# yml-bit/CTA-GAN

Hardware: AMD Instinct MI355X
Metric: paired 512x512 slices/sec (G+D step); generator rel-L2 vs CPU reference (higher is better)
Workload: dtype bf16; 1 GPU; HdGan stage-2 full G+D train step (G, Reg, STN, D_m, losses, Adam x3), 16 paired 512x512 slices/GPU; per_gpu_batch=16, global_batch=16, size=512, parallelism=single, rccl_ranks=1, dp_backend=none

## Files before the change

cta_gan_amd/csrc/conv_small.hip:

```cpp
#include <stdlib.h>
#include "common.h"
#include "ctg_knobs.h"

struct SmallArgs {
    const float* s0;
    const float* s1;
    const void* w;
    const float* bias;
    void* y;
    float* stats;
    int B, Hi, Wi, Cin, kh, kw, stride, pad, pad_mode;
    int Ho, Wo, Cout, y_ld, act, Kreal, ntiles;
};

#define SMALL_PREF 5

template <typename T, int KPAD, int BN, bool PO = false, bool X3 = false, bool KXW = false>
__global__ __launch_bounds__(256) void conv_small_kernel(const SmallArgs a) {
    static_assert(!KXW || (KPAD == 64 && sizeof(T) == 2), "kx-window layout: 8 kernel rows x 8 columns of bf16");
    static_assert(!PO || sizeof(T) == 4 || X3, "split-pair output: the fp32 or the split-bf16 instantiation");
    static_assert(!X3 || (sizeof(T) == 2 && PO), "split-bf16 MFMA: bf16 tiles, split-pair result");
    constexpr int EPC = VecOf<T>::N;
    constexpr int CPR = KPAD / EPC;
    constexpr int KCH = X3 ? 8 : (CPR < 8 ? CPR : 8);
    constexpr int NSUB = X3 ? KPAD / 32 : CPR / KCH;
    constexpr int CPRW = X3 ? 2 * CPR : CPR;
    constexpr int TM = 4, TN = BN / 16;
    constexpr int PPI = 256 / CPR;
    constexpr int A_BYTES = 256 * KPAD * (int)sizeof(T) * (X3 ? 2 : 1);
    constexpr int ST_BYTES = PO ? 256 * (BN * 4 + 16) : sizeof(T) == 2 ? 256 * (BN * 2 + 16) : 4 * BN * 2 * 4;
    constexpr int A_REGION = A_BYTES > ST_BYTES ? A_BYTES : ST_BYTES;
    typedef T OutT;
    extern __shared__ __attribute__((aligned(16))) char smem[];

    const int tid = threadIdx.x, lane = tid & 63, wave = tid >> 6;
    const int n = blockIdx.y;
    const int tx_n = (a.Wo + 15) >> 4;
    const int PH = 15 * a.stride + a.kh, PW = 15 * a.stride + a.kw;
    const int plane = PH * PW;
    const int patch_elems = a.Cin * plane;

    char* sA = smem;
    char* sW = smem + A_REGION;
    float* patch = reinterpret_cast<float*>(sW + BN * CPRW * 16);

    const int wg = xcd_contiguous(blockIdx.x, gridDim.x);
    const int q = a.ntiles / (int)gridDim.x, rem = a.ntiles % (int)gridDim.x;
    const int t_begin = wg * q + (wg < rem ? wg : rem);
    const int t_end = t_begin + q + (wg < rem ? 1 : 0);
    if (t_begin >= t_end) return;

    {
        const T* W = (const T*)a.w;
        for (int i = tid; i < BN * CPRW; i += 256) {
            const int row = i / CPRW, kc = i - row * CPRW;
            const int sub = kc / KCH, kcl = kc - sub * KCH;
            *reinterpret_cast<u32x4*>(sW + ((sub * BN + row) * KCH + swz<KCH>(row, kcl)) * 16) =
                *reinterpret_cast<const u32x4*>(W + (size_t)row * (CPRW * EPC) + kc * EPC);
        }
    }
    int pe_yx[SMALL_PREF];
#pragma unroll
    for (int j = 0; j < SMALL_PREF; ++j) {
        const int i = tid + 256 * j;
        const int c = i / plane, r = i - c * plane;
        const int py = r / PW, px = r - py * PW;
        pe_yx[j] = i < patch_elems ? (c << 30) | (py << 15) | px : -1;
    }
    float pre[SMALL_PREF];
    unsigned pre_ok = 0;
    auto fetch_patch = [&](int sp) __attribute__((always_inline)) {
        const int iy0 = (sp / tx_n) * 16 * a.stride - a.pad, ix0 = (sp % tx_n) * 16 * a.stride - a.pad;
#pragma unroll
        for (int j = 0; j < SMALL_PREF; ++j) {
            const int e = pe_yx[j];
            int iy = iy0 + ((e >> 15) & 0x7fff), ix = ix0 + (e & 0x7fff);
            if (a.pad_mode == PAD_REFLECT) { iy = reflect_idx(iy, a.Hi); ix = reflect_idx(ix, a.Wi); }
            const bool ok = e >= 0 && (unsigned)iy < (unsigned)a.Hi && (unsigned)ix < (unsigned)a.Wi;
            const float* src = (ok && ((e >> 30) & 1)) ? a.s1 : a.s0;
            const int off = ok ? iy * a.Wi + ix : 0;
            pre[j] = src[(size_t)n * a.Hi * a.Wi + off];
            pre_ok = ok ? (pre_ok | (1u << j)) : (pre_ok & ~(1u << j));
        }
    };
    const int kc = tid % CPR;
    int koff[EPC];
    unsigned kvalid = 0;
#pragma unroll
    for (int e = 0; e < EPC; ++e) {
        const int k = kc * EPC + e;
        const int kk = a.kh * a.kw;
        const int c = k / kk, r = k - c * kk;
        const int ky = r / a.kw, kx = r - ky * a.kw;
        koff[e] = k < a.Kreal ? (c * PH + ky) * PW + kx : 0;
        kvalid |= (k < a.Kreal ? 1u : 0u) << e;
    }
    const int co_l = (lane >> 4) * 4;
    OutT* __restrict__ Y = (OutT*)a.y;
    const float nslope = a.act == ACT_RELU ? 0.f : a.act == ACT_LRELU ? LRELU_SLOPE : 1.f;
    const bool raw = a.bias == nullptr && a.act == ACT_NONE;

    float bv[TN][4];
#pragma unroll
    for (int nt = 0; nt < TN; ++nt)
#pragma unroll
        for (int r = 0; r < 4; ++r) {
            const int co = nt * 16 + co_l + r;
            bv[nt][r] = (a.bias != nullptr && co < a.Cout) ? a.bias[co] : 0.f;
        }

    auto stash_patch = [&]() __attribute__((always_inline)) {
#pragma unroll
        for (int j = 0; j < SMALL_PREF; ++j)
            if (pe_yx[j] >= 0) patch[tid + 256 * j] = ((pre_ok >> j) & 1u) ? pre[j] : 0.f;
    };
    fetch_patch(t_begin);
    stash_patch();
    for (int sp = t_begin; sp < t_end; ++sp) {
        const int y0 = (sp / tx_n) * 16, x0 = (sp % tx_n) * 16;
        lds_barrier();
        if (sp + 1 < t_end) fetch_patch(sp + 1);
        if constexpr (KXW) {
            const int ky = tid & 7, grp = tid >> 3;
            const int r = grp >> 1, xh = (grp & 1) * 8;
            const bool row_ok = ky < a.kh;
            const float* prow = patch + (r + ky) * PW + xh;
            float win[16];
#pragma unroll
            for (int j = 0; j < 15; ++j) win[j] = (row_ok && j < a.kw + 7) ? prow[j] : 0.f;
            win[15] = 0.f;
            const int sub = X3 ? ky >> 2 : 0, kcl = X3 ? ky & 3 : ky;
#pragma unroll
            for (int pp = 0; pp < 8; ++pp) {
                const int p = r * 16 + xh + pp;
                float v[8];
#pragma unroll
                for (int e = 0; e < 8; ++e) v[e] = e < a.kw ? win[pp + e] : 0.f;
                if constexpr (X3) {
                    bf16x8 hi, lo;
#pragma unroll
                    for (int e = 0; e < 8; ++e) {
                        hi[e] = (bf16_t)v[e];
                        lo[e] = (bf16_t)(v[e] - (float)hi[e]);
                    }
                    *reinterpret_cast<bf16x8*>(sA + ((sub * 256 + p) * KCH + swz<KCH>(p, kcl)) * 16) = hi;
                    *reinterpret_cast<bf16x8*>(sA + ((sub * 256 + p) * KCH + swz<KCH>(p, kcl + 4)) * 16) = lo;
                } else {
                    bf16x8 o;
#pragma unroll
                    for (int e = 0; e < 8; ++e) o[e] = (bf16_t)v[e];
                    *reinterpret_cast<bf16x8*>(sA + ((sub * 256 + p) * KCH + swz<KCH>(p, kcl)) * 16) = o;
                }
            }
        } else {
            const int sub = X3 ? kc / 4 : kc / KCH, kcl = X3 ? kc & 3 : kc - sub * KCH;
#pragma unroll 2
            for (int it = 0; it < CPR; ++it) {
                const int p = tid / CPR + it * PPI;
                const int base = ((p >> 4) * a.stride) * PW + (p & 15) * a.stride;
                Chunk<T> o;
#pragma unroll
                for (int e = 0; e < EPC; ++e) {
                    const float v = patch[base + koff[e]];
                    o.v[e] = ((kvalid >> e) & 1u) ? v : 0.f;
                }
                if constexpr (X3) {
                    bf16x8 hi, lo;
#pragma unroll
                    for (int e = 0; e < 8; ++e) {
                        hi[e] = (bf16_t)o.v[e];
                        lo[e] = (bf16_t)(o.v[e] - (float)hi[e]);
                    }
                    *reinterpret_cast<bf16x8*>(sA + ((sub * 256 + p) * KCH + swz<KCH>(p, kcl)) * 16) = hi;
                    *reinterpret_cast<bf16x8*>(sA + ((sub * 256 + p) * KCH + swz<KCH>(p, kcl + 4)) * 16) = lo;
                } else {
                    o.store(reinterpret_cast<T*>(sA + ((sub * 256 + p) * KCH + swz<KCH>(p, kcl)) * 16));
                }
            }
        }
        lds_barrier();

        f32x4 acc[TM][TN];
#pragma unroll
        for (int i = 0; i < TM; ++i)
#pragma unroll
            for (int j = 0; j < TN; ++j) acc[i][j] = f32x4{0.f, 0.f, 0.f, 0.f};
#pragma unroll
        for (int sub = 0; sub < NSUB; ++sub) {
            if constexpr (X3) {
                const int c4 = lane >> 4;
                u32x4 fa[TM], fb[TN], fl[TN];
#pragma unroll
                for (int mt = 0; mt < TM; ++mt) {
                    const int row = (wave * TM + mt) * 16 + (lane & 15);
                    fa[mt] = *reinterpret_cast<const u32x4*>(sA + ((sub * 256 + row) * KCH + swz<KCH>(row, c4)) * 16);
                }
#pragma unroll
                for (int nt = 0; nt < TN; ++nt) {
                    const int row = nt * 16 + (lane & 15);
                    fb[nt] = *reinterpret_cast<const u32x4*>(sW + ((sub * BN + row) * KCH + swz<KCH>(row, c4)) * 16);
                    fl[nt] = *reinterpret_cast<const u32x4*>(sW + ((sub * BN + row) * KCH + swz<KCH>(row, c4 + 4)) * 16);
                }
#pragma unroll
                for (int mt = 0; mt < TM; ++mt)
#pragma unroll
                    for (int nt = 0; nt < TN; ++nt) {
                        acc[mt][nt] = __builtin_amdgcn_mfma_f32_16x16x32_bf16(
                            __builtin_bit_cast(bf16x8, fb[nt]), __builtin_bit_cast(bf16x8, fa[mt]), acc[mt][nt], 0, 0, 0);
                        acc[mt][nt] = __builtin_amdgcn_mfma_f32_16x16x32_bf16(
                            __builtin_bit_cast(bf16x8, fl[nt]), __builtin_bit_cast(bf16x8, fa[mt]), acc[mt][nt], 0, 0, 0);
                    }
#pragma unroll
                for (int mt = 0; mt < TM; ++mt) {
                    const int row = (wave * TM + mt) * 16 + (lane & 15);
                    fa[mt] = *reinterpret_cast<const u32x4*>(sA + ((sub * 256 + row) * KCH + swz<KCH>(row, c4 + 4)) * 16);
                }
#pragma unroll
                for (int mt = 0; mt < TM; ++mt)
#pragma unroll
                    for (int nt = 0; nt < TN; ++nt)
                        acc[mt][nt] = __builtin_amdgcn_mfma_f32_16x16x32_bf16(
                            __builtin_bit_cast(bf16x8, fb[nt]), __builtin_bit_cast(bf16x8, fa[mt]), acc[mt][nt], 0, 0, 0);
            } else
#pragma unroll
            for (int ks = 0; ks < KCH / 4; ++ks) {
                const int c4 = ks * 4 + (lane >> 4);
                u32x4 fa[TM], fb[TN];
#pragma unroll
                for (int mt = 0; mt < TM; ++mt) {
                    const int row = (wave * TM + mt) * 16 + (lane & 15);
                    fa[mt] = *reinterpret_cast<const u32x4*>(sA + ((sub * 256 + row) * KCH + swz<KCH>(row, c4)) * 16);
                }
#pragma unroll
                for (int nt = 0; nt < TN; ++nt) {
                    const int row = nt * 16 + (lane & 15);
                    fb[nt] = *reinterpret_cast<const u32x4*>(sW + ((sub * BN + row) * KCH + swz<KCH>(row, c4)) * 16);
                }
#pragma unroll
                for (int mt = 0; mt < TM; ++mt)
#pragma unroll
                    for (int nt = 0; nt < TN; ++nt) {
                        if constexpr (sizeof(T) == 2) {
                            acc[mt][nt] = __builtin_amdgcn_mfma_f32_16x16x32_bf16(
                                __builtin_bit_cast(bf16x8, fb[nt]), __builtin_bit_cast(bf16x8, fa[mt]), acc[mt][nt], 0, 0, 0);
                        } else {
                            const f32x4 va = __builtin_bit_cast(f32x4, fa[mt]);
                            const f32x4 vb = __builtin_bit_cast(f32x4, fb[nt]);
#pragma unroll
                            for (int qq = 0; qq < 4; ++qq)
                                acc[mt][nt] = __builtin_amdgcn_mfma_f32_16x16x4f32(vb[qq], va[qq], acc[mt][nt], 0, 0, 0);
                        }
                    }
            }
        }
        if (sp + 1 < t_end) stash_patch();
        lds_barrier();

        if (a.stats != nullptr) {
            float* red = reinterpret_cast<float*>(smem);
#pragma unroll
            for (int nt = 0; nt < TN; ++nt) {
                float s1[4] = {0.f, 0.f, 0.f, 0.f}, s2[4] = {0.f, 0.f, 0.f, 0.f};
#pragma unroll
                for (int mt = 0; mt < TM; ++mt) {
                    const bool valid = (y0 + wave * TM + mt < a.Ho) && (x0 + (lane & 15) < a.Wo);
#pragma unroll
                    for (int r = 0; r < 4; ++r) {
                        const float v = valid ? acc[mt][nt][r] : 0.f;
                        s1[r] += v;
                        s2[r] += v * v;
                    }
                }
#pragma unroll
                for (int r = 0; r < 4; ++r) {
                    s1[r] = row16_sum_to_lane15(s1[r]);
                    s2[r] = row16_sum_to_lane15(s2[r]);
                    if ((lane & 15) == 15) {
                        const int cl = nt * 16 + co_l + r;
                        red[(wave * BN + cl) * 2] = s1[r];
                        red[(wave * BN + cl) * 2 + 1] = s2[r];
                    }
                }
            }
            lds_barrier();
            if (tid < BN && tid < a.Cout) {
                float t1 = 0.f, t2 = 0.f;
#pragma unroll
                for (int w = 0; w < 4; ++w) { t1 += red[(w * BN + tid) * 2]; t2 += red[(w * BN + tid) * 2 + 1]; }
                float* dst = a.stats + (((size_t)n * a.ntiles + sp) * a.Cout + tid) * 2;
                dst[0] = t1;
                dst[1] = t2;
            }
            lds_barrier();
        }
        if constexpr (sizeof(OutT) == 2 && !PO) {
            constexpr int RS = BN * 2 + 16;
            char* st = smem;
#pragma unroll
            for (int nt = 0; nt < TN; ++nt) {
                const int co = nt * 16 + co_l;
#pragma unroll
                for (int mt = 0; mt < TM; ++mt) {
                    const int prow = (wave * TM + mt) * 16 + (lane & 15);
                    bf16x4 o;
                    if (raw) {
#pragma unroll
                        for (int r = 0; r < 4; ++r) o[r] = (bf16_t)acc[mt][nt][r];
                    } else {
#pragma unroll
                        for (int r = 0; r < 4; ++r) {
                            const float v = acc[mt][nt][r] + bv[nt][r];
                            o[r] = (bf16_t)(v > 0.f ? v : v * nslope);
                        }
                    }
                    *reinterpret_cast<bf16x4*>(st + prow * RS + co * 2) = o;
                }
            }
            lds_barrier();
            constexpr int CPO = BN / 8;
#pragma unroll
            for (int it = 0; it < CPO; ++it) {
                const int cidx = tid + 256 * it;
                const int prow = cidx / CPO, ch = (cidx % CPO) * 8;
                const int oy = y0 + (prow >> 4), ox = x0 + (prow & 15);
                if (oy < a.Ho && ox < a.Wo && ch < a.Cout)
                    *reinterpret_cast<u32x4*>(Y + (((size_t)n * a.Ho + oy) * a.Wo + ox) * a.y_ld + ch) =
                        *reinterpret_cast<const u32x4*>(st + prow * RS + ch * 2);
            }
        } else if constexpr (PO) {
            constexpr int RS = BN * 4 + 16;
            char* st = smem;
#pragma unroll
            for (int nt = 0; nt < TN; ++nt) {
                const int co = nt * 16 + co_l;
#pragma unroll
                for (int mt = 0; mt < TM; ++mt) {
                    const int prow = (wave * TM + mt) * 16 + (lane & 15);
                    f32x4 o;
                    if (raw) {
                        o = acc[mt][nt];
                    } else {
#pragma unroll
                        for (int r = 0; r < 4; ++r) {
                            const float v = acc[mt][nt][r] + bv[nt][r];
                            o[r] = v > 0.f ? v : v * nslope;
                        }
                    }
                    *reinterpret_cast<f32x4*>(st + prow * RS + co * 4) = o;
                }
            }
            lds_barrier();
            bf16_t* __restrict__ Yp = (bf16_t*)a.y;
            const int y_lo = a.y_ld >> 1;
            constexpr int CPO = BN / 8;
#pragma unroll
            for (int it = 0; it < CPO; ++it) {
                const int cidx = tid + 256 * it;
                const int prow = cidx / CPO, ch = (cidx % CPO) * 8;
                const int oy = y0 + (prow >> 4), ox = x0 + (prow & 15);
                if (oy < a.Ho && ox < a.Wo && ch < a.Cout) {
                    const f32x4 v0 = *reinterpret_cast<const f32x4*>(st + prow * RS + ch * 4);
                    const f32x4 v1 = *reinterpret_cast<const f32x4*>(st + prow * RS + ch * 4 + 16);
                    bf16x8 hi, lo;
#pragma unroll
                    for (int e = 0; e < 4; ++e) {
                        hi[e] = (bf16_t)v0[e];
                        lo[e] = (bf16_t)(v0[e] - (float)hi[e]);
                        hi[4 + e] = (bf16_t)v1[e];
                        lo[4 + e] = (bf16_t)(v1[e] - (float)hi[4 + e]);
                    }
                    bf16_t* yp = Yp + (((size_t)n * a.Ho + oy) * a.Wo + ox) * a.y_ld + ch;
                    *reinterpret_cast<bf16x8*>(yp) = hi;
                    *reinterpret_cast<bf16x8*>(yp + y_lo) = lo;
                }
            }
        } else {
#pragma unroll
            for (int mt = 0; mt < TM; ++mt) {
                const int oy = y0 + wave * TM + mt, ox = x0 + (lane & 15);
                if (oy >= a.Ho || ox >= a.Wo) continue;
                OutT* yp = Y + (((size_t)n * a.Ho + oy) * a.Wo + ox) * a.y_ld;
#pragma unroll
                for (int nt = 0; nt < TN; ++nt) {
                    const int co = nt * 16 + co_l;
                    if (co >= a.Cout) continue;
                    f32x4 v;
#pragma unroll
                    for (int r = 0; r < 4; ++r) {
                        const float t = acc[mt][nt][r] + bv[nt][r];
                        v[r] = t > 0.f ? t : t * nslope;
                    }
                    *reinterpret_cast<f32x4*>(yp + co) = v;
                }
            }
        }
    }
}

template <typename T, int KPAD, int BN, bool PO = false, bool X3 = false, bool KXW = false>
static int launch_small(SmallArgs& a, hipStream_t st, int* tiles_out) {
    const int PH = 15 * a.stride + a.kh, PW = 15 * a.stride + a.kw;
    if (a.Cin * PH * PW > SMALL_PREF * 256 || PH >= 32768 || PW >= 32768) return CTG_EINVAL;
    const int a_bytes = 256 * KPAD * (int)sizeof(T) * (X3 ? 2 : 1);
    const int st_bytes = PO ? 256 * (BN * 4 + 16) : sizeof(T) == 2 ? 256 * (BN * 2 + 16) : 4 * BN * 2 * 4;
    const int smem = (a_bytes > st_bytes ? a_bytes : st_bytes) + BN * KPAD * (int)sizeof(T) * (X3 ? 2 : 1) + (a.Cin * PH * PW + 4) * 4;
    if (smem > 160 * 1024) return CTG_EINVAL;
    static unsigned long long attr_mask = 0;
    if (smem > 64 * 1024) {
        const int rc = ctg_lds_attr_once((const void*)conv_small_kernel<T, KPAD, BN, PO, X3, KXW>, 160 * 1024, &attr_mask);
        if (rc != CTG_OK) return rc;
    }
    const int tiles = ((a.Ho + 15) / 16) * ((a.Wo + 15) / 16);
    a.ntiles = tiles;
    if (tiles_out != nullptr) *tiles_out = tiles;
    const int wg_total = ctg_knobs().small_wgs;
    int gx = (wg_total + a.B - 1) / a.B;
    if (gx > tiles) gx = tiles;
    hipLaunchKernelGGL((conv_small_kernel<T, KPAD, BN, PO, X3, KXW>), dim3(gx, a.B), dim3(256), smem, st, a);
    return ctg_launch_status();
}

extern "C" int ctg_conv_smallcin(int dtype, const float* s0, const float* s1, int Cin, int B, int Hi, int Wi, int kh,
                                 int kw, int stride, int pad, int pad_mode, const void* w, int w_npad, int Kpad, int w_layout,
                                 const float* bias, int act, void* y, int y_ld, int Ho, int Wo, int Cout,
                                 float* stats_part, int* stats_slabs_out, void* stream) {
    CTG_ENTER();
    if (w_layout != 0 && (w_layout != 1 || Cin != 1 || stride != 1 || kh > 8 || kw > 8 || Kpad != 64 || Cout <= 32 ||
                          dtype == DT_F32)) return CTG_EINVAL;
    if (dtype != DT_F32 && dtype != DT_BF16 && dtype != DT_PAIR) return CTG_EINVAL;
    const bool pair = dtype == DT_PAIR;
    if (pair && (Cout % 8 || y_ld % 16 || y_ld < 2 * Cout)) return CTG_EINVAL;
    const int epc = dtype == DT_BF16 ? 8 : 4;
    if (Cin < 1 || Cin > 2 || (Cin == 2 && s1 == nullptr) || s0 == nullptr || w == nullptr || y == nullptr) return CTG_EINVAL;
    if (B < 1 || kh < 1 || kw < 1 || stride < 1 || stride > 2 || pad < 0) return CTG_EINVAL;
    if (act != ACT_NONE && act != ACT_RELU && act != ACT_LRELU) return CTG_EINVAL;
    if ((w_layout == 0 && Cin * kh * kw > Kpad) || (Kpad != 32 && Kpad != 64)) return CTG_EINVAL;
    if (Cout < 1 || Cout > 64 || Cout % epc || y_ld % epc || y_ld < Cout) return CTG_EINVAL;
    if (pad_mode == PAD_REFLECT && (pad >= Hi || pad >= Wi)) return CTG_EINVAL;
    if (Ho != (Hi + 2 * pad - kh) / stride + 1 || Wo != (Wi + 2 * pad - kw) / stride + 1 || Ho < 1 || Wo < 1) return CTG_EINVAL;
    const int bn = Cout > 32 ? 64 : 32;
    if (w_npad < bn) return CTG_EINVAL;
    if (((uintptr_t)w & 15) || ((uintptr_t)y & 15)) return CTG_EINVAL;
    SmallArgs a;
    a.s0 = s0; a.s1 = s1; a.w = w; a.bias = bias; a.y = y; a.stats = stats_part;
    a.B = B; a.Hi = Hi; a.Wi = Wi; a.Cin = Cin; a.kh = kh; a.kw = kw; a.stride = stride; a.pad = pad;
    a.pad_mode = pad_mode; a.Ho = Ho; a.Wo = Wo; a.Cout = Cout; a.y_ld = y_ld; a.act = act; a.Kreal = Cin * kh * kw;
    hipStream_t st = (hipStream_t)stream;
    int tiles = 0, rc;
    if (w_layout == 1) {
        rc = pair ? launch_small<bf16_t, 64, 64, true, true, true>(a, st, &tiles) : launch_small<bf16_t, 64, 64, false, false, true>(a, st, &tiles);
    } else if (dtype == DT_BF16) {
        if (Kpad == 64) rc = bn == 64 ? launch_small<bf16_t, 64, 64>(a, st, &tiles) : launch_small<bf16_t, 64, 32>(a, st, &tiles);
        else rc = bn == 64 ? launch_small<bf16_t, 32, 64>(a, st, &tiles) : launch_small<bf16_t, 32, 32>(a, st, &tiles);
    } else if (pair) {
        if (Kpad == 64) rc = bn == 64 ? launch_small<bf16_t, 64, 64, true, true>(a, st, &tiles) : launch_small<bf16_t, 64, 32, true, true>(a, st, &tiles);
        else rc = bn == 64 ? launch_small<bf16_t, 32, 64, true, true>(a, st, &tiles) : launch_small<bf16_t, 32, 32, true, true>(a, st, &tiles);
    } else {
        if (Kpad == 64) rc = bn == 64 ? launch_small<float, 64, 64>(a, st, &tiles) : launch_small<float, 64, 32>(a, st, &tiles);
        else rc = bn == 64 ? launch_small<float, 32, 64>(a, st, &tiles) : launch_small<float, 32, 32>(a, st, &tiles);
    }
    if (stats_slabs_out != nullptr) *stats_slabs_out = stats_part != nullptr ? tiles : 0;
    return rc;
}
```

cta_gan_amd/csrc/loss_stn.hip:

```cpp
#include "common.h"

static inline int ew_blocks(long items) {
    long b = (items + 255) / 256;
    return (int)(b < 1 ? 1 : (b > 4096 ? 4096 : b));
}

__device__ __forceinline__ void block_partial(float v, float* __restrict__ part) {
    __shared__ float ws[4];
    v = wave_sum(v);
    if ((threadIdx.x & 63) == 0) ws[threadIdx.x >> 6] = v;
    __syncthreads();
    if (threadIdx.x == 0) part[blockIdx.x] = (ws[0] + ws[1]) + (ws[2] + ws[3]);
}

__global__ __launch_bounds__(256) void sum_finalize_kernel(const float* __restrict__ part, int n, float scale,
                                                           float* __restrict__ out, int accumulate) {
    __shared__ double ws[4];
    double s = 0.0;
    for (int i = threadIdx.x; i < n; i += 256) s += (double)part[i];
#pragma unroll
    for (int o = 32; o > 0; o >>= 1) s += __shfl_xor(s, o, 64);
    if ((threadIdx.x & 63) == 0) ws[threadIdx.x >> 6] = s;
    __syncthreads();
    if (threadIdx.x == 0) {
        const float r = (float)(((ws[0] + ws[1]) + (ws[2] + ws[3])) * (double)scale);
        out[0] = accumulate ? out[0] + r : r;
    }
}

struct WarpGeom {
    float iy, ix, my, mx;
};

__device__ __forceinline__ void warp_coord(float g, float f, int size, float& c, float& mult) {
    const float sm1 = (float)(size - 1);
    float loc = g + f;
    loc = 2.f * (loc / sm1 - 0.5f);
    float u = ((loc + 1.f) / 2.f) * sm1;
    float m = sm1 / 2.f;
    if (u <= 0.f) { u = 0.f; m = 0.f; }
    else if (u >= sm1) { u = sm1; m = 0.f; }
    c = u;
    mult = (m * 2.f) / sm1;
}

__global__ void warp_fwd_kernel(const float* __restrict__ src, const float* __restrict__ flow, long fs_n, long fs_c,
                                long fs_y, long fs_x, float* __restrict__ out, int B, int H, int W) {
    const long total = (long)B * H * W;
    for (long i = (long)blockIdx.x * blockDim.x + threadIdx.x; i < total; i += (long)gridDim.x * blockDim.x) {
        const int x = (int)(i % W);
        const int y = (int)((i / W) % H);
        const int n = (int)(i / ((long)W * H));
        const float* fl = flow + n * fs_n + y * fs_y + x * fs_x;
        float iy, ix, my, mx;
        warp_coord((float)y, fl[0], H, iy, my);
        warp_coord((float)x, fl[fs_c], W, ix, mx);
        const float fy = floorf(iy), fx = floorf(ix);
        const int y0 = (int)fy, x0 = (int)fx, y1 = y0 + 1, x1 = x0 + 1;
        const float nw = ((fx + 1.f) - ix) * ((fy + 1.f) - iy), ne = (ix - fx) * ((fy + 1.f) - iy);
        const float sw = ((fx + 1.f) - ix) * (iy - fy), se = (ix - fx) * (iy - fy);
        const float* s = src + (size_t)n * H * W;
        float r = s[(size_t)y0 * W + x0] * nw;
        if (x1 < W) r += s[(size_t)y0 * W + x1] * ne;
        if (y1 < H) r += s[(size_t)y1 * W + x0] * sw;
        if (y1 < H && x1 < W) r += s[(size_t)y1 * W + x1] * se;
        out[i] = r;
    }
}

__global__ void zero_f32_kernel(float* __restrict__ p, long n) {
    for (long i = (long)blockIdx.x * blockDim.x + threadIdx.x; i < n; i += (long)gridDim.x * blockDim.x) p[i] = 0.f;
}

__global__ void warp_bwd_kernel(const float* __restrict__ src, const float* __restrict__ flow, long fs_n, long fs_c,
                                long fs_y, long fs_x, const float* __restrict__ gout, float* __restrict__ dsrc,
                                float* __restrict__ dflow, int B, int H, int W) {
    const long total = (long)B * H * W;
    for (long i = (long)blockIdx.x * blockDim.x + threadIdx.x; i < total; i += (long)gridDim.x * blockDim.x) {
        const int x = (int)(i % W);
        const int y = (int)((i / W) % H);
        const int n = (int)(i / ((long)W * H));
        const long fo = n * fs_n + y * fs_y + x * fs_x;
        float iy, ix, my, mx;
        warp_coord((float)y, flow[fo], H, iy, my);
        warp_coord((float)x, flow[fo + fs_c], W, ix, mx);
        const float fy = floorf(iy), fx = floorf(ix);
        const int y0 = (int)fy, x0 = (int)fx, y1 = y0 + 1, x1 = x0 + 1;
        const float wx1 = ix - fx, wx0 = (fx + 1.f) - ix, wy1 = iy - fy, wy0 = (fy + 1.f) - iy;
        const float g = gout[i];
        const float* s = src + (size_t)n * H * W;
        float* ds = dsrc ? dsrc + (size_t)n * H * W : nullptr;
        const bool bx = x1 < W, by = y1 < H;
        const float vnw = s[(size_t)y0 * W + x0];
        const float vne = bx ? s[(size_t)y0 * W + x1] : 0.f;
        const float vsw = by ? s[(size_t)y1 * W + x0] : 0.f;
        const float vse = (bx && by) ? s[(size_t)y1 * W + x1] : 0.f;
        if (ds) {
            atomicAdd(ds + (size_t)y0 * W + x0, wx0 * wy0 * g);
            if (bx) atomicAdd(ds + (size_t)y0 * W + x1, wx1 * wy0 * g);
            if (by) atomicAdd(ds + (size_t)y1 * W + x0, wx0 * wy1 * g);
            if (bx && by) atomicAdd(ds + (size_t)y1 * W + x1, wx1 * wy1 * g);
        }
        if (dflow) {
            const float gix = (-vnw * wy0 + vne * wy0 - vsw * wy1 + vse * wy1) * g;
            const float giy = (-vnw * wx0 - vne * wx1 + vsw * wx0 + vse * wx1) * g;
            dflow[fo] = my * giy;
            dflow[fo + fs_c] = mx * gix;
        }
    }
}

__global__ void warp_det_prep_kernel(const float* __restrict__ gout, long long* __restrict__ acc, unsigned* __restrict__ maxbits,
                                     long n) {
    unsigned m = 0u;
    for (long i = (long)blockIdx.x * blockDim.x + threadIdx.x; i < n; i += (long)gridDim.x * blockDim.x) {
        acc[i] = 0;
        const unsigned b = __float_as_uint(gout[i]) & 0x7fffffffu;
        m = b > m ? b : m;
    }
#pragma unroll
    for (int o = 32; o > 0; o >>= 1) {
        const unsigned t = (unsigned)__shfl_xor((int)m, o, 64);
        m = t > m ? t : m;
    }
    if ((threadIdx.x & 63) == 0 && m) atomicMax(maxbits, m);
}

__device__ __forceinline__ float det_scale(unsigned maxbits, bool inverse) {
    int e = (int)(maxbits >> 23) - 127;
    e = e < -88 ? -88 : (e > 88 ? 88 : e);
    return __uint_as_float((unsigned)((inverse ? e - 38 : 38 - e) + 127) << 23);
}

__global__ void warp_bwd_det_kernel(const float* __restrict__ flow, long fs_n, long fs_c, long fs_y, long fs_x,
                                    const float* __restrict__ gout, long long* __restrict__ acc,
                                    const unsigned* __restrict__ maxbits, int B, int H, int W) {
    const long total = (long)B * H * W;
    const float sc = det_scale(maxbits[0], false);
    for (long i = (long)blockIdx.x * blockDim.x + threadIdx.x; i < total; i += (long)gridDim.x * blockDim.x) {
        const int x = (int)(i % W);
        const int y = (int)((i / W) % H);
        const int n = (int)(i / ((long)W * H));
        const long fo = n * fs_n + y * fs_y + x * fs_x;
        float iy, ix, my, mx;
        warp_coord((float)y, flow[fo], H, iy, my);
        warp_coord((float)x, flow[fo + fs_c], W, ix, mx);
        const float fy = floorf(iy), fx = floorf(ix);
        const int y0 = (int)fy, x0 = (int)fx, y1 = y0 + 1, x1 = x0 + 1;
        const float wx1 = ix - fx, wx0 = (fx + 1.f) - ix, wy1 = iy - fy, wy0 = (fy + 1.f) - iy;
        const float g = gout[i] * sc;
        unsigned long long* ds = reinterpret_cast<unsigned long long*>(acc + (size_t)n * H * W);
        const bool bx = x1 < W, by = y1 < H;
        atomicAdd(ds + (size_t)y0 * W + x0, (unsigned long long)__float2ll_rn(wx0 * wy0 * g));
        if (bx) atomicAdd(ds + (size_t)y0 * W + x1, (unsigned long long)__float2ll_rn(wx1 * wy0 * g));
        if (by) atomicAdd(ds + (size_t)y1 * W + x0, (unsigned long long)__float2ll_rn(wx0 * wy1 * g));
        if (bx && by) atomicAdd(ds + (size_t)y1 * W + x1, (unsigned long long)__float2ll_rn(wx1 * wy1 * g));
    }
}

__global__ void warp_det_finish_kernel(const long long* __restrict__ acc, const unsigned* __restrict__ maxbits,
                                       float* __restrict__ dsrc, long n) {
    const float inv = det_scale(maxbits[0], true);
    for (long i = (long)blockIdx.x * blockDim.x + threadIdx.x; i < n; i += (long)gridDim.x * blockDim.x)
        dsrc[i] = (float)acc[i] * inv;
}

__global__ void smooth_fwd_kernel(const float* __restrict__ f, long sn, long sc, long sy, long sx, int B, int C,
                                  int H, int W, float inv_nx, float inv_ny, float* __restrict__ part) {
    const long total = (long)B * C * H * W;
    float acc = 0.f;
    for (long i = (long)blockIdx.x * blockDim.x + threadIdx.x; i < total; i += (long)gridDim.x * blockDim.x) {
        const int x = (int)(i % W);
        const int y = (int)((i / W) % H);
        const int c = (int)((i / ((long)W * H)) % C);
        const int n = (int)(i / ((long)W * H * C));
        const float* p = f + n * sn + c * sc + y * sy + x * sx;
        const float v = p[0];
        if (x + 1 < W) { const float d = p[sx] - v; acc += d * d * inv_nx; }
        if (y + 1 < H) { const float d = p[sy] - v; acc += d * d * inv_ny; }
    }
    block_partial(acc, part);
}

__global__ void smooth_bwd_kernel(const float* __restrict__ f, long sn, long sc, long sy, long sx, int B, int C,
                                  int H, int W, float inv_nx, float inv_ny, const float* __restrict__ gscale,
                                  float* __restrict__ df, int accumulate) {
    const long total = (long)B * C * H * W;
    const float g = gscale[0];
    for (long i = (long)blockIdx.x * blockDim.x + threadIdx.x; i < total; i += (long)gridDim.x * blockDim.x) {
        const int x = (int)(i % W);
        const int y = (int)((i / W) % H);
        const int c = (int)((i / ((long)W * H)) % C);
        const int n = (int)(i / ((long)W * H * C));
        const long o = n * sn + c * sc + y * sy + x * sx;
        const float v = f[o];
        float r = 0.f;
        if (x + 1 < W) r -= 2.f * (f[o + sx] - v) * inv_nx;
        if (x > 0) r += 2.f * (v - f[o - sx]) * inv_nx;
        if (y + 1 < H) r -= 2.f * (f[o + sy] - v) * inv_ny;
        if (y > 0) r += 2.f * (v - f[o - sy]) * inv_ny;
        df[o] = accumulate ? df[o] + g * r : g * r;
    }
}

__device__ __forceinline__ float l1_term(float a, float b, const float* mask, long i, float& dsign) {
    if (mask == nullptr) {
        const float d = a - b;
        dsign = d > 0.f ? 1.f : (d < 0.f ? -1.f : 0.f);
        return fabsf(d);
    }
    const float bb = mask[i] < 0.3f ? 0.f : 1.f;
    float bm = b * bb;
    if (bm == 0.f) bm = -1.f;
    const float ab = a * bb;
    const float am = ab == 0.f ? -1.f : ab;
    const float d = am - bm;
    dsign = ab == 0.f ? 0.f : bb * (d > 0.f ? 1.f : (d < 0.f ? -1.f : 0.f));
    return fabsf(d);
}

__global__ void l1_fwd_kernel(const float* __restrict__ a, const float* __restrict__ b,
                              const float* __restrict__ mask, long n, float* __restrict__ part) {
    float acc = 0.f;
    for (long i = (long)blockIdx.x * blockDim.x + threadIdx.x; i < n; i += (long)gridDim.x * blockDim.x) {
        float ds;
        acc += l1_term(a[i], b[i], mask, i, ds);
    }
    block_partial(acc, part);
}

__global__ void l1_bwd_kernel(const float* __restrict__ a, const float* __restrict__ b,
                              const float* __restrict__ mask, long n, const float* __restrict__ gscale, float inv_n,
                              float* __restrict__ da, int accumulate) {
    const float g = gscale[0] * inv_n;
    for (long i = (long)blockIdx.x * blockDim.x + threadIdx.x; i < n; i += (long)gridDim.x * blockDim.x) {
        float ds;
        l1_term(a[i], b[i], mask, i, ds);
        da[i] = accumulate ? da[i] + g * ds : g * ds;
    }
}

__global__ void avgpool_fwd_kernel(const float* __restrict__ x, int HW, float* __restrict__ out) {
    __shared__ float ws[4];
    const int n = blockIdx.x;
    float acc = 0.f;
    for (int i = threadIdx.x; i < HW; i += blockDim.x) acc += x[(size_t)n * HW + i];
    acc = wave_sum(acc);
    if ((threadIdx.x & 63) == 0) ws[threadIdx.x >> 6] = acc;
    __syncthreads();
    if (threadIdx.x == 0) out[n] = ((ws[0] + ws[1]) + (ws[2] + ws[3])) / (float)HW;
}

__global__ void avgpool_bwd_kernel(const float* __restrict__ gout, int HW, float* __restrict__ dx, long total) {
    for (long i = (long)blockIdx.x * blockDim.x + threadIdx.x; i < total; i += (long)gridDim.x * blockDim.x)
        dx[i] = gout[i / HW] / (float)HW;
}

__device__ __forceinline__ double gan_term(double p, double t, int mode) {
    if (mode == 0) return (p - t) * (p - t);
    const double lp = fmax(log(p), -100.0), lq = fmax(log(1.0 - p), -100.0);
    return -(t * lp + (1.0 - t) * lq);
}
__device__ __forceinline__ float gan_term_grad(float p, float t, int mode) {
    if (mode == 0) return 2.f * (p - t);
    return (p - t) / fmaxf(p * (1.f - p), 1e-12f);
}

__global__ __launch_bounds__(256) void lsgan_finalize_kernel(const float* __restrict__ pooled, int B, int nb, float t0,
                                                             float s0, float t1, float s1, int mode,
                                                             float* __restrict__ out) {
    __shared__ double ws[4];
    double s = 0.0;
    for (int b = threadIdx.x; b < B; b += 256)
        s += (double)(b < nb ? s0 : s1) * gan_term((double)pooled[b], (double)(b < nb ? t0 : t1), mode);
#pragma unroll
    for (int o = 32; o > 0; o >>= 1) s += __shfl_xor(s, o, 64);
    if ((threadIdx.x & 63) == 0) ws[threadIdx.x >> 6] = s;
    __syncthreads();
    if (threadIdx.x == 0) out[0] = (float)((ws[0] + ws[1]) + (ws[2] + ws[3]));
}

__global__ void lsgan_bwd_kernel(const float* __restrict__ pooled, int HW, int nb, float t0, float s0, float t1, float s1,
                                 int mode, const float* __restrict__ gscale, float* __restrict__ dx, long total) {
    const float g = gscale[0] / (float)HW;
    for (long i = (long)blockIdx.x * blockDim.x + threadIdx.x; i < total; i += (long)gridDim.x * blockDim.x) {
        const int b = (int)(i / HW);
        dx[i] = g * (b < nb ? s0 : s1) * gan_term_grad(pooled[b], b < nb ? t0 : t1, mode);
    }
}

struct ScalarList { const float* p[8]; int n; };
__global__ void sum_scalars_kernel(const ScalarList L, float* __restrict__ out) {
    float s = 0.f;
    for (int i = 0; i < L.n; ++i) s += L.p[i][0];
    out[0] = s;
}

__global__ void act_bwd_sum_kernel(const float* __restrict__ g, const float* __restrict__ y, int act,
                                   float* __restrict__ out, long n, float* __restrict__ part) {
    float acc = 0.f;
    for (long i = (long)blockIdx.x * blockDim.x + threadIdx.x; i < n; i += (long)gridDim.x * blockDim.x) {
        const float v = g[i] * act_grad_from_out(y[i], act);
        out[i] = v;
        acc += v;
    }
    block_partial(acc, part);
}

template <typename T>
__global__ void weight_pack_kernel(const float* __restrict__ src, long sn, long sk, long stp, int Nreal, int Kreal,
                                   T* __restrict__ dst, int ntaps, int Npad, int Kpad) {
    const long total = (long)ntaps * Npad * Kpad;
    for (long i = (long)blockIdx.x * blockDim.x + threadIdx.x; i < total; i += (long)gridDim.x * blockDim.x) {
        const int k = (int)(i % Kpad);
        const int n = (int)((i / Kpad) % Npad);
        const int t = (int)(i / ((long)Kpad * Npad));
        const float v = (n < Nreal && k < Kreal) ? src[n * sn + k * sk + t * stp] : 0.f;
        st1(dst + i, v);
    }
}

#define PACK_MAX_T 24
struct PackList {
    const float* src[PACK_MAX_T];
    void* dst[PACK_MAX_T];
    long sn[PACK_MAX_T], sk[PACK_MAX_T], stp[PACK_MAX_T];
    int nreal[PACK_MAX_T], kreal[PACK_MAX_T], ntaps[PACK_MAX_T], npad[PACK_MAX_T], kpad[PACK_MAX_T];
    int first[PACK_MAX_T + 1];
    int count;
};
#define PACK_CHUNK 2048

template <typename T>
__global__ __launch_bounds__(256) void weight_pack_multi_kernel(const PackList L) {
    int j = 0;
    while (j + 1 < L.count && (int)blockIdx.x >= L.first[j + 1]) ++j;
    const int Kpad = L.kpad[j], Npad = L.npad[j], Nreal = L.nreal[j], Kreal = L.kreal[j];
    const long sn = L.sn[j], sk = L.sk[j], stp = L.stp[j];
    const float* __restrict__ src = L.src[j];
    T* __restrict__ dst = (T*)L.dst[j];
    const unsigned total = (unsigned)L.ntaps[j] * Npad * Kpad;
    const unsigned base = ((unsigned)blockIdx.x - L.first[j]) * PACK_CHUNK;
#pragma unroll 2
    for (unsigned e = threadIdx.x; e < PACK_CHUNK; e += 256) {
        const unsigned i = base + e;
        if (i >= total) break;
        const unsigned k = i % (unsigned)Kpad, r = i / (unsigned)Kpad;
        const unsigned n = r % (unsigned)Npad, t = r / (unsigned)Npad;
        const float v = ((int)n < Nreal && (int)k < Kreal) ? src[n * sn + k * sk + t * stp] : 0.f;
        st1(dst + i, v);
    }
}

#define ADAM_MAX_T 24
struct AdamList {
    float* p[ADAM_MAX_T];
    const float* g[ADAM_MAX_T];
    float* m[ADAM_MAX_T];
    float* v[ADAM_MAX_T];
    int n[ADAM_MAX_T];
    int count;
};
#define ADAM_CHUNK 4096

__global__ __launch_bounds__(256) void adam_kernel(const AdamList L, float lr, float b1, float b2, float eps,
                                                   float bc1, float bc2_sqrt, const float* __restrict__ dev_bc) {
    if (dev_bc != nullptr) {
        bc1 = dev_bc[1];
        bc2_sqrt = dev_bc[2];
    }
    const int t = blockIdx.y;
    if (t >= L.count) return;
    const int n = L.n[t];
    const int beg = blockIdx.x * ADAM_CHUNK;
    if (beg >= n) return;
    const int end = min(beg + ADAM_CHUNK, n);
    float* __restrict__ p = L.p[t];
    const float* __restrict__ g = L.g[t];
    float* __restrict__ m = L.m[t];
    float* __restrict__ v = L.v[t];
    const float step = lr / bc1;
    for (int i = beg + threadIdx.x; i < end; i += 256) {
        const float gi = g[i];
        float mi = m[i], vi = v[i];
        mi = mi + (gi - mi) * (1.f - b1);
        vi = vi * b2 + (1.f - b2) * gi * gi;
        const float denom = sqrtf(vi) / bc2_sqrt + eps;
        p[i] = p[i] - step * (mi / denom);
        m[i] = mi;
        v[i] = vi;
    }
}

__global__ void adam_tick_kernel(float* __restrict__ state, float b1, float b2) {
    if (threadIdx.x == 0 && blockIdx.x == 0) {
        const double step = (double)state[0] + 1.0;
        state[0] = (float)step;
        state[1] = (float)(1.0 - pow((double)b1, step));
        state[2] = (float)sqrt(1.0 - pow((double)b2, step));
    }
}

extern "C" int ctg_warp_fwd(const float* src, const float* flow, long fs_n, long fs_c, long fs_y, long fs_x,
                            float* out, int B, int H, int W, void* stream) {
    CTG_ENTER();
    if (H < 2 || W < 2) return CTG_EINVAL;
    hipLaunchKernelGGL(warp_fwd_kernel, dim3(ew_blocks((long)B * H * W)), dim3(256), 0, (hipStream_t)stream, src,
                       flow, fs_n, fs_c, fs_y, fs_x, out, B, H, W);
    return ctg_launch_status();
}

extern "C" int ctg_warp_bwd(const float* src, const float* flow, long fs_n, long fs_c, long fs_y, long fs_x,
                            const float* gout, float* dsrc, float* dflow, int B, int H, int W, void* det_ws, void* stream) {
    CTG_ENTER();
    if (H < 2 || W < 2) return CTG_EINVAL;
    hipStream_t st = (hipStream_t)stream;
    if (dsrc && det_ws) {
        if ((uintptr_t)det_ws & 7) return CTG_EINVAL;
        const long n = (long)B * H * W;
        long long* acc = (long long*)det_ws;
        unsigned* maxbits = (unsigned*)(acc + n);
        hipLaunchKernelGGL(zero_f32_kernel, dim3(1), dim3(64), 0, st, (float*)maxbits, 2L);
        hipLaunchKernelGGL(warp_det_prep_kernel, dim3(ew_blocks(n)), dim3(256), 0, st, gout, acc, maxbits, n);
        hipLaunchKernelGGL(warp_bwd_det_kernel, dim3(ew_blocks(n)), dim3(256), 0, st, flow, fs_n, fs_c, fs_y, fs_x, gout, acc,
                           maxbits, B, H, W);
        hipLaunchKernelGGL(warp_det_finish_kernel, dim3(ew_blocks(n)), dim3(256), 0, st, acc, maxbits, dsrc, n);
        if (dflow)
            hipLaunchKernelGGL(warp_bwd_kernel, dim3(ew_blocks(n)), dim3(256), 0, st, src, flow, fs_n, fs_c, fs_y, fs_x, gout,
                               (float*)nullptr, dflow, B, H, W);
        return ctg_launch_status();
    }
    if (dsrc) {
        hipLaunchKernelGGL(zero_f32_kernel, dim3(ew_blocks((long)B * H * W / 4 + 1)), dim3(256), 0, st, dsrc, (long)B * H * W);
    }
    hipLaunchKernelGGL(warp_bwd_kernel, dim3(ew_blocks((long)B * H * W)), dim3(256), 0, st, src, flow, fs_n, fs_c,
                       fs_y, fs_x, gout, dsrc, dflow, B, H, W);
    return ctg_launch_status();
}

extern "C" int ctg_smooth_fwd(const float* f, long sn, long sc, long sy, long sx, int B, int C, int H, int W,
                              float weight, float* part, float* out, void* stream) {
    CTG_ENTER();
    if (H < 2 || W < 2) return CTG_EINVAL;
    const long total = (long)B * C * H * W;
    const int nb = ew_blocks(total);
    const float inv_nx = 1.f / (float)((long)B * C * H * (W - 1)), inv_ny = 1.f / (float)((long)B * C * (H - 1) * W);
    hipStream_t st = (hipStream_t)stream;
    hipLaunchKernelGGL(smooth_fwd_kernel, dim3(nb), dim3(256), 0, st, f, sn, sc, sy, sx, B, C, H, W, inv_nx, inv_ny,
                       part);
    hipLaunchKernelGGL(sum_finalize_kernel, dim3(1), dim3(256), 0, st, (const float*)part, nb, weight, out, 0);
    return ctg_launch_status();
}

extern "C" int ctg_smooth_bwd(const float* f, long sn, long sc, long sy, long sx, int B, int C, int H, int W,
                              float weight, const float* gscale, float* df, int accumulate, void* stream) {
    CTG_ENTER();
    if (H < 2 || W < 2) return CTG_EINVAL;
    const long total = (long)B * C * H * W;
    const float inv_nx = weight / (float)((long)B * C * H * (W - 1)), inv_ny = weight / (float)((long)B * C * (H - 1) * W);
    hipLaunchKernelGGL(smooth_bwd_kernel, dim3(ew_blocks(total)), dim3(256), 0, (hipStream_t)stream, f, sn, sc, sy, sx,
                       B, C, H, W, inv_nx, inv_ny, gscale, df, accumulate);
    return ctg_launch_status();
}

extern "C" int ctg_l1_fwd(const float* a, const float* b, const float* mask, long n, float weight, float* part,
                          float* out, void* stream) {
    CTG_ENTER();
    if (n < 1) return CTG_EINVAL;
    const int nb = ew_blocks(n);
    hipStream_t st = (hipStream_t)stream;
    hipLaunchKernelGGL(l1_fwd_kernel, dim3(nb), dim3(256), 0, st, a, b, mask, n, part);
    hipLaunchKernelGGL(sum_finalize_kernel, dim3(1), dim3(256), 0, st, (const float*)part, nb, weight / (float)n, out, 0);
    return ctg_launch_status();
}

extern "C" int ctg_l1_bwd(const float* a, const float* b, const float* mask, long n, float weight, const float* gscale,
                          float* da, int accumulate, void* stream) {
    CTG_ENTER();
    if (n < 1) return CTG_EINVAL;
    hipLaunchKernelGGL(l1_bwd_kernel, dim3(ew_blocks(n)), dim3(256), 0, (hipStream_t)stream, a, b, mask, n, gscale,
                       weight / (float)n, da, accumulate);
    return ctg_launch_status();
}

extern "C" int ctg_avgpool_fwd(const float* x, int B, int HW, float* out, void* stream) {
    CTG_ENTER();
    if (B < 1 || HW < 1) return CTG_EINVAL;
    hipLaunchKernelGGL(avgpool_fwd_kernel, dim3(B), dim3(256), 0, (hipStream_t)stream, x, HW, out);
    return ctg_launch_status();
}

extern "C" int ctg_lsgan_fwd(const float* x, int B, int HW, int nb, float t0, float s0, float t1, float s1, int mode,
                             float* pooled, float* out, void* stream) {
    CTG_ENTER();
    if (B < 1 || HW < 1 || nb < 0 || nb > B || (mode != 0 && mode != 1)) return CTG_EINVAL;
    hipStream_t st = (hipStream_t)stream;
    hipLaunchKernelGGL(avgpool_fwd_kernel, dim3(B), dim3(256), 0, st, x, HW, pooled);
    hipLaunchKernelGGL(lsgan_finalize_kernel, dim3(1), dim3(256), 0, st, (const float*)pooled, B, nb, t0, s0, t1, s1, mode, out);
    return ctg_launch_status();
}

extern "C" int ctg_lsgan_bwd(const float* pooled, int B, int HW, int nb, float t0, float s0, float t1, float s1, int mode,
                             const float* gscale, float* dx, void* stream) {
    CTG_ENTER();
    if (B < 1 || HW < 1 || nb < 0 || nb > B || (mode != 0 && mode != 1)) return CTG_EINVAL;
    const long total = (long)B * HW;
    hipLaunchKernelGGL(lsgan_bwd_kernel, dim3(ew_blocks(total)), dim3(256), 0, (hipStream_t)stream, pooled, HW, nb, t0, s0,
                       t1, s1, mode, gscale, dx, total);
    return ctg_launch_status();
}

extern "C" int ctg_sum_scalars(int count, const void* const* scalars, float* out, void* stream) {
    CTG_ENTER();
    if (count < 1 || count > 8) return CTG_EINVAL;
    ScalarList L;
    for (int i = 0; i < 8; ++i) L.p[i] = i < count ? (const float*)scalars[i] : nullptr;
    L.n = count;
    hipLaunchKernelGGL(sum_scalars_kernel, dim3(1), dim3(1), 0, (hipStream_t)stream, L, out);
    return ctg_launch_status();
}

extern "C" int ctg_act_bwd_sum_f32(const float* g, const float* y, int act, float* out, long n, float* part, float* sum_out,
                                   int accumulate, void* stream) {
    CTG_ENTER();
    if (n < 1 || g == nullptr || y == nullptr || out == nullptr || part == nullptr || sum_out == nullptr) return CTG_EINVAL;
    const int nb = ew_blocks(n);
    hipStream_t st = (hipStream_t)stream;
    hipLaunchKernelGGL(act_bwd_sum_kernel, dim3(nb), dim3(256), 0, st, g, y, act, out, n, part);
    hipLaunchKernelGGL(sum_finalize_kernel, dim3(1), dim3(256), 0, st, (const float*)part, nb, 1.f, sum_out, accumulate);
    return ctg_launch_status();
}

extern "C" int ctg_avgpool_bwd(const float* gout, int B, int HW, float* dx, void* stream) {
    CTG_ENTER();
    if (B < 1 || HW < 1) return CTG_EINVAL;
    const long total = (long)B * HW;
    hipLaunchKernelGGL(avgpool_bwd_kernel, dim3(ew_blocks(total)), dim3(256), 0, (hipStream_t)stream, gout, HW, dx,
                       total);
    return ctg_launch_status();
}

extern "C" int ctg_weight_pack(int dtype, const float* src, long sn, long sk, long stp, int Nreal, int Kreal,
                               void* dst, int ntaps, int Npad, int Kpad, void* stream) {
    CTG_ENTER();
    if (Nreal > Npad || Kreal > Kpad || ntaps < 1) return CTG_EINVAL;
    const long total = (long)ntaps * Npad * Kpad;
    hipStream_t st = (hipStream_t)stream;
    if (dtype == DT_BF16)
        hipLaunchKernelGGL((weight_pack_kernel<bf16_t>), dim3(ew_blocks(total)), dim3(256), 0, st, src, sn, sk, stp,
                           Nreal, Kreal, (bf16_t*)dst, ntaps, Npad, Kpad);
    else if (dtype == DT_F32)
        hipLaunchKernelGGL((weight_pack_kernel<float>), dim3(ew_blocks(total)), dim3(256), 0, st, src, sn, sk, stp,
                           Nreal, Kreal, (float*)dst, ntaps, Npad, Kpad);
    else return CTG_EINVAL;
    return ctg_launch_status();
}

extern "C" int ctg_weight_pack_multi(int dtype, int count, const void* const* src, void* const* dst, const long* sn,
                                     const long* sk, const long* stp, const int* nreal, const int* kreal,
                                     const int* ntaps, const int* npad, const int* kpad, void* stream) {
    CTG_ENTER();
    if (count < 0 || (dtype != DT_BF16 && dtype != DT_F32)) return CTG_EINVAL;
    hipStream_t st = (hipStream_t)stream;
    for (int base = 0; base < count; base += PACK_MAX_T) {
        PackList L;
        L.count = count - base < PACK_MAX_T ? count - base : PACK_MAX_T;
        int blocks = 0;
        for (int i = 0; i < L.count; ++i) {
            const int q = base + i;
            if (nreal[q] > npad[q] || kreal[q] > kpad[q] || ntaps[q] < 1 || src[q] == nullptr || dst[q] == nullptr) return CTG_EINVAL;
            const long total = (long)ntaps[q] * npad[q] * kpad[q];
            if (total >= (1L << 31)) return CTG_EINVAL;
            L.src[i] = (const float*)src[q]; L.dst[i] = dst[q];
            L.sn[i] = sn[q]; L.sk[i] = sk[q]; L.stp[i] = stp[q];
            L.nreal[i] = nreal[q]; L.kreal[i] = kreal[q]; L.ntaps[i] = ntaps[q]; L.npad[i] = npad[q]; L.kpad[i] = kpad[q];
            L.first[i] = blocks;
            blocks += (int)((total + PACK_CHUNK - 1) / PACK_CHUNK);
        }
        L.first[L.count] = blocks;
        if (blocks == 0) continue;
        if (dtype == DT_BF16) hipLaunchKernelGGL((weight_pack_multi_kernel<bf16_t>), dim3(blocks), dim3(256), 0, st, L);
        else hipLaunchKernelGGL((weight_pack_multi_kernel<float>), dim3(blocks), dim3(256), 0, st, L);
    }
    return ctg_launch_status();
}

extern "C" int ctg_adam_tick(float* state3, float beta1, float beta2, void* stream) {
    CTG_ENTER();
    if (state3 == nullptr) return CTG_EINVAL;
    hipLaunchKernelGGL(adam_tick_kernel, dim3(1), dim3(64), 0, (hipStream_t)stream, state3, beta1, beta2);
    return ctg_launch_status();
}

extern "C" int ctg_adam_step(int count, void* const* params, const void* const* grads, void* const* exp_avg,
                             void* const* exp_avg_sq, const long* numel, float lr, float beta1, float beta2, float eps,
                             int step, const float* dev_state3, void* stream) {
    CTG_ENTER();
    if (count < 0 || (step < 1 && dev_state3 == nullptr)) return CTG_EINVAL;
    if (step < 1) step = 1;
    const double bc1 = 1.0 - pow((double)beta1, (double)step);
    const double bc2 = 1.0 - pow((double)beta2, (double)step);
    hipStream_t st = (hipStream_t)stream;
    for (int base = 0; base < count; base += ADAM_MAX_T) {
        AdamList L;
        L.count = count - base < ADAM_MAX_T ? count - base : ADAM_MAX_T;
        long maxn = 0;
        for (int i = 0; i < L.count; ++i) {
            if (numel[base + i] > 0x7fffffffL) return CTG_EINVAL;
            L.p[i] = (float*)params[base + i];
            L.g[i] = (const float*)grads[base + i];
            L.m[i] = (float*)exp_avg[base + i];
            L.v[i] = (float*)exp_avg_sq[base + i];
            L.n[i] = (int)numel[base + i];
            if (numel[base + i] > maxn) maxn = numel[base + i];
        }
        if (maxn == 0) continue;
        dim3 grid((unsigned)((maxn + ADAM_CHUNK - 1) / ADAM_CHUNK), L.count);
        hipLaunchKernelGGL(adam_kernel, grid, dim3(256), 0, st, L, lr, beta1, beta2, eps, (float)bc1,
                           (float)sqrt(bc2), dev_state3);
    }
    return ctg_launch_status();
}
```

Baseline: 355.4 slices/s.

## Use shifted-row LDS layout for kx-window conv, cap grid to occupancy, vectorise det prep

For the non-split bf16 kx-window conv path, the kernel now builds per-row bf16 shifted copies of the input patch in LDS (23 rows x 16 positions) and reads MFMA A-fragments directly from them, replacing the per-thread im2col expansion. It also skips the unused patch prefetch slots. The bf16 conv launcher caps the workgroup count at the number of resident blocks, using a cached occupancy query. Separately, the warp-backward deterministic prep kernel is vectorised to 16-byte loads and stores, launched with fewer blocks, and issues one atomic per block instead of one per wave.

```diff
diff --git a/cta_gan_amd/csrc/conv_small.hip b/cta_gan_amd/csrc/conv_small.hip
--- a/cta_gan_amd/csrc/conv_small.hip
+++ b/cta_gan_amd/csrc/conv_small.hip
@@ -30,6 +30,8 @@
     constexpr int A_BYTES = 256 * KPAD * (int)sizeof(T) * (X3 ? 2 : 1);
     constexpr int ST_BYTES = PO ? 256 * (BN * 4 + 16) : sizeof(T) == 2 ? 256 * (BN * 2 + 16) : 4 * BN * 2 * 4;
     constexpr int A_REGION = A_BYTES > ST_BYTES ? A_BYTES : ST_BYTES;
+    constexpr int SH_ROWS = 23;
+    static_assert(SH_ROWS * 256 <= A_REGION, "the shifted copies live where the im2col tile would");
     typedef T OutT;
     extern __shared__ __attribute__((aligned(16))) char smem[];
 
@@ -73,6 +75,7 @@
         const int iy0 = (sp / tx_n) * 16 * a.stride - a.pad, ix0 = (sp % tx_n) * 16 * a.stride - a.pad;
 #pragma unroll
         for (int j = 0; j < SMALL_PREF; ++j) {
+            if (KXW && !X3 && 256 * j >= patch_elems) continue;
             const int e = pe_yx[j];
             int iy = iy0 + ((e >> 15) & 0x7fff), ix = ix0 + (e & 0x7fff);
             if (a.pad_mode == PAD_REFLECT) { iy = reflect_idx(iy, a.Hi); ix = reflect_idx(ix, a.Wi); }
@@ -120,7 +123,28 @@
         const int y0 = (sp / tx_n) * 16, x0 = (sp % tx_n) * 16;
         lds_barrier();
         if (sp + 1 < t_end) fetch_patch(sp + 1);
-        if constexpr (KXW) {
+        if constexpr (KXW && !X3) {
+            if (tid < SH_ROWS * 8) {
+                const int R = tid >> 3, p0 = (tid & 7) * 2;
+                const bool row_ok = R < PH;
+                float win[9];
+#pragma unroll
+                for (int j = 0; j < 9; ++j) {
+                    const bool ok = row_ok && p0 + j < PW;
+                    const float v = patch[ok ? R * PW + p0 + j : 0];
+                    win[j] = ok ? v : 0.f;
+                }
+                bf16_t b[9];
+#pragma unroll
+                for (int j = 0; j < 9; ++j) b[j] = (bf16_t)win[j];
+                bf16x8 o0, o1;
+#pragma unroll
+                for (int e = 0; e < 8; ++e) { o0[e] = b[e]; o1[e] = b[e + 1]; }
+                bf16x8* dst = reinterpret_cast<bf16x8*>(sA + (R * 16 + p0) * 16);
+                dst[0] = o0;
+                dst[1] = o1;
+            }
+        } else if constexpr (KXW) {
             const int ky = tid & 7, grp = tid >> 3;
             const int r = grp >> 1, xh = (grp & 1) * 8;
             const bool row_ok = ky < a.kh;
@@ -228,8 +252,12 @@
                 u32x4 fa[TM], fb[TN];
 #pragma unroll
                 for (int mt = 0; mt < TM; ++mt) {
-                    const int row = (wave * TM + mt) * 16 + (lane & 15);
-                    fa[mt] = *reinterpret_cast<const u32x4*>(sA + ((sub * 256 + row) * KCH + swz<KCH>(row, c4)) * 16);
+                    if constexpr (KXW) {
+                        fa[mt] = *reinterpret_cast<const u32x4*>(sA + ((wave * TM + mt + c4) * 16 + (lane & 15)) * 16);
+                    } else {
+                        const int row = (wave * TM + mt) * 16 + (lane & 15);
+                        fa[mt] = *reinterpret_cast<const u32x4*>(sA + ((sub * 256 + row) * KCH + swz<KCH>(row, c4)) * 16);
+                    }
                 }
 #pragma unroll
                 for (int nt = 0; nt < TN; ++nt) {
@@ -413,7 +441,22 @@
     const int tiles = ((a.Ho + 15) / 16) * ((a.Wo + 15) / 16);
     a.ntiles = tiles;
     if (tiles_out != nullptr) *tiles_out = tiles;
-    const int wg_total = ctg_knobs().small_wgs;
+    int wg_total = ctg_knobs().small_wgs;
+    if constexpr (sizeof(T) == 2 && !PO) {
+        static int occ_dev[64];
+        int dev = 0;
+        if (hipGetDevice(&dev) != hipSuccess) dev = 0;
+        dev &= 63;
+        if (occ_dev[dev] == 0) {
+            int occ = 0;
+            if (hipOccupancyMaxActiveBlocksPerMultiprocessor(&occ, (const void*)conv_small_kernel<T, KPAD, BN, PO, X3, KXW>, 256,
+                                                             smem) != hipSuccess || occ < 1)
+                occ = 1 << 20;
+            occ_dev[dev] = occ;
+        }
+        const long resident = (long)occ_dev[dev] * ctg_cu_count();
+        if (resident < wg_total) wg_total = (int)resident;
+    }
     int gx = (wg_total + a.B - 1) / a.B;
     if (gx > tiles) gx = tiles;
     hipLaunchKernelGGL((conv_small_kernel<T, KPAD, BN, PO, X3, KXW>), dim3(gx, a.B), dim3(256), smem, st, a);
diff --git a/cta_gan_amd/csrc/loss_stn.hip b/cta_gan_amd/csrc/loss_stn.hip
--- a/cta_gan_amd/csrc/loss_stn.hip
+++ b/cta_gan_amd/csrc/loss_stn.hip
@@ -110,10 +110,23 @@
     }
 }
 
-__global__ void warp_det_prep_kernel(const float* __restrict__ gout, long long* __restrict__ acc, unsigned* __restrict__ maxbits,
-                                     long n) {
+__global__ __launch_bounds__(256) void warp_det_prep_kernel(const float* __restrict__ gout, long long* __restrict__ acc,
+                                                            unsigned* __restrict__ maxbits, long n, long n4) {
+    __shared__ unsigned wave_max[4];
     unsigned m = 0u;
-    for (long i = (long)blockIdx.x * blockDim.x + threadIdx.x; i < n; i += (long)gridDim.x * blockDim.x) {
+    const long stride = (long)gridDim.x * blockDim.x;
+    for (long i = (long)blockIdx.x * blockDim.x + threadIdx.x; i < n4; i += stride) {
+        const u32x4 g = *reinterpret_cast<const u32x4*>(gout + 4 * i);
+        u32x4* z = reinterpret_cast<u32x4*>(acc + 4 * i);
+        z[0] = u32x4{0u, 0u, 0u, 0u};
+        z[1] = u32x4{0u, 0u, 0u, 0u};
+#pragma unroll
+        for (int e = 0; e < 4; ++e) {
+            const unsigned b = g[e] & 0x7fffffffu;
+            m = b > m ? b : m;
+        }
+    }
+    for (long i = 4 * n4 + (long)blockIdx.x * blockDim.x + threadIdx.x; i < n; i += stride) {
         acc[i] = 0;
         const unsigned b = __float_as_uint(gout[i]) & 0x7fffffffu;
         m = b > m ? b : m;
@@ -123,7 +136,18 @@
         const unsigned t = (unsigned)__shfl_xor((int)m, o, 64);
         m = t > m ? t : m;
     }
-    if ((threadIdx.x & 63) == 0 && m) atomicMax(maxbits, m);
+    if ((threadIdx.x & 63) == 0) wave_max[threadIdx.x >> 6] = m;
+    __syncthreads();
+    if (threadIdx.x == 0) {
+#pragma unroll
+        for (int w = 1; w < 4; ++w) m = wave_max[w] > m ? wave_max[w] : m;
+        if (m) atomicMax(maxbits, m);
+    }
+}
+
+static inline int det_prep_blocks(long n) {
+    long b = (n + 1023) / 1024;
+    return (int)(b < 1 ? 1 : (b > 1024 ? 1024 : b));
 }
 
 __device__ __forceinline__ float det_scale(unsigned maxbits, bool inverse) {
@@ -421,7 +445,8 @@
         long long* acc = (long long*)det_ws;
         unsigned* maxbits = (unsigned*)(acc + n);
         hipLaunchKernelGGL(zero_f32_kernel, dim3(1), dim3(64), 0, st, (float*)maxbits, 2L);
-        hipLaunchKernelGGL(warp_det_prep_kernel, dim3(ew_blocks(n)), dim3(256), 0, st, gout, acc, maxbits, n);
+        const long n4 = (((uintptr_t)gout | (uintptr_t)acc) & 15) ? 0 : n / 4;
+        hipLaunchKernelGGL(warp_det_prep_kernel, dim3(det_prep_blocks(n)), dim3(256), 0, st, gout, acc, maxbits, n, n4);
         hipLaunchKernelGGL(warp_bwd_det_kernel, dim3(ew_blocks(n)), dim3(256), 0, st, flow, fs_n, fs_c, fs_y, fs_x, gout, acc,
                            maxbits, B, H, W);
         hipLaunchKernelGGL(warp_det_finish_kernel, dim3(ew_blocks(n)), dim3(256), 0, st, acc, maxbits, dsrc, n);
```

New measurement: 357.6 slices/s, median of 6. Within noise of the previous version (+0.6%).
